# rhysnewell/Lorikeet

Hardware: AMD Instinct MI355X
Metric: PairHMM cell-updates/s (GCUPS) (higher is better)
Workload: dtype f64; 1 GPU; config2 x 1024 regions per GPU: 128 reads x 8 haps, R=150, H=300; regions_per_gpu=1024, seed=1000, env=PHMM_REGION_OWN_QUEUE=0 in this process only

## Files before the change

### lorikeet_amd/csrc/phmm_chain_kernels.hip

```cpp
#include "phmm_device.hpp"

namespace phmm {

namespace {

#ifndef PHMM_CHAIN_L
#define PHMM_CHAIN_L 16
#endif
constexpr int CL = PHMM_CHAIN_L;
#ifndef PHMM_RING
#define PHMM_RING 256
#endif
constexpr int RING = PHMM_RING;
constexpr int RING_SLOTS = RING + 4 + 1;
constexpr int CHAIN_META = CHAIN_MAX_READS + 8;
constexpr uint32_t X_PAD = 0x100u;
constexpr uint32_t X_NONE = 0x102u;
constexpr int LEAD = CL - 1;

__device__ __forceinline__ double from_left_inject(double v, double inject, bool group_head) {
    constexpr int ctrl = CL == 16 ? 0x111 : 0x138;
    int lo = __builtin_amdgcn_update_dpp(__double2loint(inject), __double2loint(v), ctrl, 0xf, 0xf, false);
    int hi = __builtin_amdgcn_update_dpp(__double2hiint(inject), __double2hiint(v), ctrl, 0xf, 0xf, false);
    if constexpr (CL == 32) {
        lo = group_head ? __double2loint(inject) : lo;
        hi = group_head ? __double2hiint(inject) : hi;
    }
    return __hiloint2double(hi, lo);
}

template <int K>
__device__ __forceinline__ void chain_fallback(const ForwardParams &p, const ChainItem &it, RowConst *ring, int lane,
                                               int grp, int l, const HapCols<K> &hc, int H, bool hv, int a, int Nh) {
    const uint32_t reg = it.region;
    for (uint32_t r = it.read_begin; r < it.read_end; ++r) {
        const uint32_t ro = p.read_off[r];
        const int R = (int)(p.read_off[r + 1] - ro);
        bool z = false;
        for (int row = lane; row < R; row += WAVE) z |= row_blocks_prescale(p, ro + row);
        const bool scaled = __ballot(z) == 0ull;
        const bool staged = R + 1 <= RING;
        lds_wave_sync();
        if (staged) {
            if (lane == 0) ring[0] = neutral_row();
            for (int row = lane; row < R; row += WAVE) ring[row + 1] = make_row(p, ro, row, R, scaled);
        }
        lds_wave_sync();
        const double scale0 = (scaled && R > 0) ? 1.0 - p.eps[p.gcp[ro]] : 1.0;
        const double fin = (scaled && R > 0) ? 1.0 - p.eps[p.base_q[ro + R - 1]] : 1.0;
        const double c0 = p.initial_condition / (double)H * scale0;
        const bool group_head = (CL == 32) && (lane == 32);
        double s = staged ? sweep_general<CL, K>(LdsView{ring}, R, l, group_head, hc, H, c0, scaled, fin)
                          : sweep_general<CL, K>(GlobalRowView{p, ro, R, scaled}, R, l, group_head, hc, H, c0, scaled, fin);
#pragma unroll
        for (int off = CL / 2; off > 0; off >>= 1) s += __shfl_xor(s, off, WAVE);
        if (l == 0 && hv) {
            const double v = log10(s) - p.initial_condition_log10;
            p.out[p.out_off[reg] + (uint64_t)(r - p.region_read_off[reg]) * (uint64_t)Nh + a] = v;
            if (const uint32_t sb = status_bits(v)) atomicOr(p.status, sb);
        }
    }
    (void)grp;
}

template <int K>
__device__ __forceinline__ void chain_fallback_streams(const ForwardParams &p, uint32_t reg, uint32_t r_begin, int n_mine,
                                                       int n_iter, int lane, int l, const HapCols<K> &hc, int H, bool hv,
                                                       int a, int Nh) {
    const uint64_t group_bits = 0xffffull << (lane & ~15);
    for (int i = 0; i < n_iter; ++i) {
        const bool valid = i < n_mine;
        const uint32_t r = r_begin + (uint32_t)i;
        const uint32_t ro = valid ? p.read_off[r] : 0u;
        const int R = valid ? (int)(p.read_off[r + 1] - ro) : 0;
        bool z = false;
        for (int row = l; row < R; row += 16) z |= row_blocks_prescale(p, ro + row);
        const bool scaled = (__ballot(z) & group_bits) == 0ull;
        const double scale0 = (scaled && R > 0) ? 1.0 - p.eps[p.gcp[ro]] : 1.0;
        const double fin = (scaled && R > 0) ? 1.0 - p.eps[p.base_q[ro + R - 1]] : 1.0;
        const double c0 = p.initial_condition / (double)H * scale0;
        double s = sweep_general<16, K>(GlobalRowView{p, ro, R, scaled}, R, l, false, hc, H, c0, scaled, fin);
#pragma unroll
        for (int off = 8; off > 0; off >>= 1) s += __shfl_xor(s, off, WAVE);
        if (l == 0 && hv && valid) {
            const double v = log10(s) - p.initial_condition_log10;
            p.out[p.out_off[reg] + (uint64_t)(r - p.region_read_off[reg]) * (uint64_t)Nh + a] = v;
            if (const uint32_t sb = status_bits(v)) atomicOr(p.status, sb);
        }
    }
}

}

template <int CLT, int K, int MODE = CHAIN_PLAIN>
__device__ __forceinline__ void chain_body(const ForwardParams &p, const ChainItem it, unsigned char *smem, const ChainItemX *x = nullptr,
                                           double *park = nullptr) {
    static_assert(CLT == CL, "one lanes-per-pair value per compilation unit");
    static_assert(MODE == CHAIN_PLAIN || CL == 16, "prefix sharing: 16 lanes per pair");
    const int col0 = MODE == CHAIN_SUFFIX ? (int)x->mask_or_col0 : 0;
    const uint32_t park_rows = MODE == CHAIN_PLAIN ? 0u : 16u * x->park_rows16;
    const uint32_t park_mask = MODE == CHAIN_PARK ? (uint32_t)x->mask_or_col0 : 0u;
    const int lane = threadIdx.x;
    const int grp = lane / CL, l = lane % CL;
    const bool group_head = (CL == 32) && (lane == 32);
    const uint32_t reg = it.region;
    const int n_chain = (int)(it.read_end - it.read_begin);
    const uint32_t h0 = p.region_hap_off[reg];
    const int Nh = (int)(p.region_hap_off[reg + 1] - h0);
    const int S = (CL == 16) ? (int)it.streams : 1;
    const int GS = (WAVE / CL) / S;
    const int sid = grp / GS;
    const int a = MODE == CHAIN_PLAIN ? (int)it.quad * GS + grp % GS : (int)x->hap[grp & 3];
    const bool hv = a < Nh;
    const int n_sub = (n_chain + S - 1) / S;
    const int TPS = (RING / 4) / S;
    const int NM = RING / S - 1;
    auto n_of = [&](int s) { return max(0, min(n_sub, n_chain - s * n_sub)); };
    const int n_mine = n_of(sid);
    uint32_t ho = 0;
    int H = 0;
    if (hv) {
        ho = p.hap_off[h0 + a];
        H = (int)(p.hap_off[h0 + a + 1] - ho);
    }
    RowConst *ring = reinterpret_cast<RowConst *>(smem);
    uint32_t *roff = reinterpret_cast<uint32_t *>(ring + RING_SLOTS);
    uint32_t *stot = roff + CHAIN_META;

    HapCols<K> hc;
    bool lane_n = false;
#pragma unroll
    for (int w = 0; w < HapCols<K>::W; ++w) hc.y[w] = 0u;
#pragma unroll
    for (int k = 0; k < K; ++k) {
        const int col = col0 + l * K + k;
        uint32_t y = col < H ? (uint32_t)p.hap_bases[ho + col] : X_PAD;
        const bool is_n = (y == 'N');
        lane_n |= is_n;
        hc.set(k, y);
    }

    const uint32_t rb = it.read_begin;
    const uint32_t byte0 = p.read_off[rb];
    const uint32_t bytes = p.read_off[it.read_end] - byte0;
    bool z = false;
    for (uint32_t i = lane; i < bytes; i += WAVE) z |= row_blocks_prescale(p, byte0 + i);
    if ((__ballot(z) | __ballot(lane_n)) != 0ull) {
        if constexpr (MODE == CHAIN_SUFFIX) {
            for (uint32_t r = rb + (uint32_t)l; r < it.read_end && hv; r += CL)
                p.out[p.out_off[reg] + (uint64_t)(r - p.region_read_off[reg]) * (uint64_t)Nh + a] = __longlong_as_double(0x7ff8000000000000ll);
            if (lane == 0) atomicOr(p.status, STATUS_RESCUE);
            return;
        }
        if (S == 1)
            chain_fallback<K>(p, it, ring, lane, grp, l, hc, H, hv, a, Nh);
        else if constexpr (CL == 16)
            chain_fallback_streams<K>(p, reg, rb + (uint32_t)(sid * n_sub), n_mine, n_sub, lane, l, hc, H, hv, a, Nh);
        return;
    }
    {
        const int sj = lane / n_sub, ij = lane % n_sub;
        uint32_t len = lane < n_chain ? p.read_off[rb + lane + 1] - p.read_off[rb + lane] + 2u : 0u;
        uint32_t incl = len;
#pragma unroll
        for (int off = 1; off < WAVE; off <<= 1) {
            const uint32_t v = __shfl_up(incl, off, WAVE);
            if (lane >= off) incl += v;
        }
        const uint32_t before = __shfl(incl, max(sj * n_sub - 1, 0), WAVE);
        const int cb = sj * (n_sub + 1);
        if (lane < 4) stot[lane] = 0u;
        if (lane < n_chain) {
            roff[cb + ij] = p.read_off[rb + lane];
            if (ij + 1 == n_of(sj)) {
                roff[cb + ij + 1] = p.read_off[rb + lane + 1];
                stot[sj] = incl - (sj > 0 ? before : 0u);
            }
        }
        if (lane == 0) ring[RING_SLOTS - 1] = neutral_row();
    }
    lds_wave_sync();
    const int S_max = (int)max(max(stot[0], stot[1]), max(stot[2], stot[3]));
    const double c_unit = ldexp(1.0, 1010);

    uint32_t pb_x = 0, pb_q = 0, pb_qp = 0, pb_i = 0, pb_d = 0, pb_dp = 0, pb_g = 0, pb_gn = 0;
    double pb_bM = 0.0, pb_bD = 0.0;
    int p_Q = 0;
    const bool producer = lane < S * TPS;
    const int ps = producer ? lane / TPS : 0, pj = lane % TPS;
    const int pcb = ps * (n_sub + 1), pn = n_of(ps);
    int p_lo = 0, p_row = pj - LEAD - TPS;
    p_Q = pj - TPS;
    uint32_t p_ro = pn > 0 ? roff[pcb] : 0u;
    int p_R = pn > 0 ? (int)(roff[pcb + 1] - p_ro) : 0;
    auto advance = [&]() {
        p_row += TPS;
        p_Q += TPS;
        while (p_lo < pn && p_row >= p_R + 2) {
            p_row -= p_R + 2;
            ++p_lo;
            if (p_lo < pn) {
                p_ro = roff[pcb + p_lo];
                p_R = (int)(roff[pcb + p_lo + 1] - p_ro);
            }
        }
    };
    auto issue = [&]() {
        advance();
        const int row = p_row, R = p_R;
        const uint32_t ro = p_ro;
        if constexpr (MODE == CHAIN_SUFFIX) {
            if (producer && p_lo < pn && row >= 0 && (uint32_t)p_Q < park_rows) {
                const double *at = park + 2 * ((size_t)x->park_row0 + (size_t)p_Q);
                pb_bM = at[0];
                pb_bD = at[1];
            }
        }
        if (producer && p_lo < pn && row >= 0 && row <= R) {
            pb_qp = row > 0 ? (uint32_t)p.base_q[ro + row - 1] : 0u;
            if (row < R) {
                pb_x = p.read_bases[ro + row];
                pb_q = p.base_q[ro + row];
                pb_i = p.ins_q[ro + row];
                pb_d = p.del_q[ro + row];
                pb_dp = row > 0 ? (uint32_t)p.del_q[ro + row - 1] : 0u;
                pb_g = p.gcp[ro + row];
                pb_gn = row + 1 < R ? (uint32_t)p.gcp[ro + row + 1] : 0u;
            }
        }
    };
    auto finish = [&](int Q0) {
        const int Q = Q0 + pj;
        const int lo = p_lo, row = p_row, R = p_R;
        RowConst n;
        if (lo < pn && row >= 0) {
            if (row < R) {
                n = make_row_bytes(p, pb_x, pb_q, pb_qp, pb_i, pb_d, pb_dp, pb_g, pb_gn, row == 0, row + 1 >= R, true);
            } else if (row == R) {
                n.mm = 1.0 - p.eps[pb_qp]; n.bI = n.mm; n.gI = 1.0; n.dDp = 0.0; n.dd = 1.0; n.pm = 1.0; n.px = 1.0;
                n.x = X_PAD; n.pad0 = (uint32_t)lo; n.pad1 = 0.0;
            } else {
                n.mm = 0.0; n.bI = 0.0; n.gI = 0.0; n.dDp = 0.0; n.dd = 1.0; n.pm = 0.0; n.px = 0.0;
                n.x = X_NONE; n.pad0 = 0;
                n.pad1 = c_unit * (lo + 1 < pn ? 1.0 - p.eps[p.gcp[roff[pcb + lo + 1]]] : 1.0);
            }
            if constexpr (MODE == CHAIN_SUFFIX) {
                n.pm = pb_bM;
                n.pad1 = pb_bD;
            }
        } else {
            n = neutral_row();
        }
        if (producer) {
            const int slot = ps * (NM + 2) + (Q & NM);
            ring[slot] = n;
            if ((Q & NM) == 0) ring[slot + NM + 1] = n;
        }
    };
    issue();
    finish(0);
    issue();
    finish(TPS);
    issue();
    finish(2 * TPS);
    lds_wave_sync();
    issue();

    const double c0 = c_unit * (n_mine > 0 ? 1.0 - p.eps[p.gcp[roff[sid * (n_sub + 1)]]] : 1.0);
    double Mp[K], Ip[K], Dp[K];
#pragma unroll
    for (int k = 0; k < K; ++k) {
        Mp[k] = 0.0;
        Ip[k] = 0.0;
        Dp[k] = c0;
    }
    double aM, aI, aD, bM = 0.0, bI = 0.0, bD = c0;
    const int edge_lane = (H > col0 ? H - 1 - col0 : 0) / K, edge_k = (H > col0 ? H - 1 - col0 : 0) % K;
    const bool last_lane = (l == edge_lane);
    const uint32_t sum_code = last_lane ? X_PAD : 0xffffffffu;
    const double log10_scale = log10(c_unit) + log10((double)H);
    auto emit = [&](const RowConst &c) {
        {
            if (last_lane && c.x == X_PAD && hv) {
                const uint32_t r = rb + (uint32_t)(sid * n_sub) + c.pad0;
                int ek = edge_k;
                asm volatile("" : "+v"(ek));
                double sum = 0.0;
#pragma unroll
                for (int k = 0; k < K; ++k)
                    if (k == ek) sum = (Dp[k] + Mp[k]) + Ip[k];
                const double v = log10(sum) - log10_scale;
                p.out[p.out_off[reg] + (uint64_t)(r - p.region_read_off[reg]) * (uint64_t)Nh + a] = v;
                if (const uint32_t sb = status_bits(v)) atomicOr(p.status, sb);
            }
        }
    };

    int q = LEAD - l;
    const int my_ring = sid * (NM + 2);
    const uint32_t my_rows = (uint32_t)(uintptr_t)(ring + my_ring);
    RowConst cA = lds_row(ring, my_ring + (q & NM)), cB;
    int q1 = q + 1;
    const int T = (S_max + CL - 1 + 1) & ~1;
    bool park_lane = false;
    double2 *park_at = nullptr;
    if constexpr (MODE == CHAIN_PARK) {
        park_lane = grp == 0 && ((park_mask >> l) & 1u) != 0u && hv && (uint32_t)(q + T) <= park_rows;
        const int b = __popc(park_mask & ((1u << l) - 1u));
        park_at = reinterpret_cast<double2 *>(park) + ((size_t)x->park_row0 + (size_t)b * park_rows + (size_t)q);
    }
    const int phase = (int)((blockIdx.x * 2654435761u) >> 26) & (TPS - 2);
    for (int t0 = 0, t1 = min(T, TPS - phase), tick = 0; t0 < T; t0 = t1, t1 = min(T, t1 + TPS), ++tick) {
        if (tick >= 1) {
            finish(TPS * tick + 2 * TPS);
            lds_wave_sync();
            issue();
        }
        for (int t = t0; t < t1; t += 2) {
            uint32_t pair_at;
            asm("v_mad_u32_u24 %0, %1, %2, %3" : "=v"(pair_at) : "v"((uint32_t)(q1 & NM)), "s"((uint32_t)sizeof(RowConst)), "v"(my_rows));
            cB = lds_row_at(pair_at, 0);
            if constexpr (MODE == CHAIN_SUFFIX) {
                aI = from_left_inject(Ip[K - 1], fma(bM, cA.bI, bI * cA.gI), group_head);
                aM = from_left_inject(Mp[K - 1], cA.pm, group_head);
            } else {
                aM = from_left<CL>(Mp[K - 1], group_head);
                aI = from_left<CL>(Ip[K - 1], group_head);
            }
            aD = from_left_inject(Dp[K - 1], cA.pad1, group_head);
            row_update<K, ROW_FAST_EXEC>(Mp, Ip, Dp, bM, bI, bD, aM, aD, cA, hc, 1.0);
            if constexpr (MODE == CHAIN_PARK)
                if (park_lane) park_at[0] = make_double2(Mp[K - 1], Dp[K - 1]);
            if (__ballot(cA.x == sum_code) != 0ull) emit(cA);
            cA = lds_row_at(pair_at, 1);
            if constexpr (MODE == CHAIN_SUFFIX) {
                bI = from_left_inject(Ip[K - 1], fma(aM, cB.bI, aI * cB.gI), group_head);
                bM = from_left_inject(Mp[K - 1], cB.pm, group_head);
            } else {
                bM = from_left<CL>(Mp[K - 1], group_head);
                bI = from_left<CL>(Ip[K - 1], group_head);
            }
            bD = from_left_inject(Dp[K - 1], cB.pad1, group_head);
            row_update<K, ROW_FAST_EXEC>(Mp, Ip, Dp, aM, aI, aD, bM, bD, cB, hc, 1.0);
            if constexpr (MODE == CHAIN_PARK) {
                if (park_lane) park_at[1] = make_double2(Mp[K - 1], Dp[K - 1]);
                park_at += 2;
            }
            if (__ballot(cB.x == sum_code) != 0ull) emit(cB);
            q1 += 2;
        }
    }
}


#define PHMM_CHAIN_K_LIST(X) \
    X(2) X(3) X(4) X(5) X(6) X(7) X(8) X(9) X(10) X(11) X(12) X(13) X(14) X(15) X(16) X(17) X(18) X(19) X(20) X(21) X(22) \
    X(23) X(24) X(25)

template <int CLT, int KLO, int KHI>
__global__ __launch_bounds__(WAVE, 2) void phmm_forward_chain(const ChainParams cp) {
    extern __shared__ __attribute__((aligned(16))) unsigned char smem[];
    const ChainItem it = cp.items[blockIdx.x];
    switch (__builtin_amdgcn_readfirstlane((int)it.k)) {
#define PHMM_CASE(KK)                                                  \
    case KK:                                                           \
        if constexpr (KK >= KLO && KK <= KHI) chain_body<CLT, KK>(cp.f, it, smem); \
        break;
        PHMM_CHAIN_K_LIST(PHMM_CASE)
#undef PHMM_CASE
        default:
            break;
    }
}

template <int CLT, int K>
__global__ __launch_bounds__(WAVE, 2) void phmm_forward_chain_k(const ChainParams cp) {
    extern __shared__ __attribute__((aligned(16))) unsigned char smem[];
    chain_body<CLT, K>(cp.f, cp.items[blockIdx.x], smem);
}

#define PHMM_CHAIN_CAT2(a, b) a##b
#define PHMM_CHAIN_CAT(a, b) PHMM_CHAIN_CAT2(a, b)
#define PHMM_CHAIN_LAUNCH PHMM_CHAIN_CAT(launch_chain_L, PHMM_CHAIN_L)

hipError_t PHMM_CHAIN_LAUNCH(int single_k, const ChainParams &cp, hipStream_t stream) {
    const size_t lds = (size_t)RING_SLOTS * sizeof(RowConst) + (CHAIN_META + 4) * sizeof(uint32_t);
#define PHMM_CASE(KK)                                                                                     \
    if (single_k == KK) {                                                                                 \
        hipLaunchKernelGGL((phmm_forward_chain_k<CL, KK>), dim3(cp.n_items), dim3(WAVE), lds, stream, cp); \
        return hipGetLastError();                                                                         \
    }
    PHMM_CHAIN_K_LIST(PHMM_CASE)
#undef PHMM_CASE
#define PHMM_RANGE(R, LO, HI)                                                                                       \
    if (single_k == -(R + 1)) {                                                                                     \
        hipLaunchKernelGGL((phmm_forward_chain<CL, LO, HI>), dim3(cp.n_items), dim3(WAVE), lds, stream, cp);        \
        return hipGetLastError();                                                                                   \
    }
    PHMM_CHAIN_RANGES(PHMM_RANGE)
#undef PHMM_RANGE
    return hipErrorInvalidValue;
}

#if PHMM_CHAIN_L == 16
hipError_t launch_chain_L32(int single_k, const ChainParams &cp, hipStream_t stream);
hipError_t launch_chain_L64(int single_k, const ChainParams &cp, hipStream_t stream);
int chain_max_k() { return 25; }
hipError_t launch_chain(int L, int single_k, const ChainParams &cp, hipStream_t stream) {
    if (!cp.n_items) return hipSuccess;
    return L == 16 ? launch_chain_L16(single_k, cp, stream) : L == 32 ? launch_chain_L32(single_k, cp, stream)
         : L == 64 ? launch_chain_L64(single_k, cp, stream) : hipErrorInvalidValue;
}
#endif

}
```

Baseline: 4555 GCUPS.

## Batch chain result emission into per-lane parked slots and flush once per wave

Row-end results are no longer written immediately with a divergent log10 and global store per emission. Each result's sum and tag are now compacted into per-lane registers via readlane, and the whole batch is flushed when the slots fill or the chain ends. The flush does the log10, the output store and the status atomic across many lanes in one go. When all active lanes share the same edge column, a uniform switch selects the column directly instead of scanning all K columns. The aim is to take serialized epilogue work out of the inner recurrence loop, at the cost of extra registers, readlane sequences and some added code size.

```diff
diff --git a/lorikeet_amd/csrc/phmm_chain_kernels.hip b/lorikeet_amd/csrc/phmm_chain_kernels.hip
--- a/lorikeet_amd/csrc/phmm_chain_kernels.hip
+++ b/lorikeet_amd/csrc/phmm_chain_kernels.hip
@@ -17,6 +17,10 @@
 constexpr uint32_t X_PAD = 0x100u;
 constexpr uint32_t X_NONE = 0x102u;
 constexpr int LEAD = CL - 1;
+constexpr int PARK_SLOTS = WAVE;
+constexpr size_t CHAIN_LDS = (size_t)RING_SLOTS * sizeof(RowConst) + (CHAIN_META + 4) * sizeof(uint32_t);
+static_assert(8 * CHAIN_LDS <= 160 * 1024, "two waves per SIMD");
+static_assert(CHAIN_MAX_READS <= 64, "a parked result names its read in six bits");
 
 __device__ __forceinline__ double from_left_inject(double v, double inject, bool group_head) {
     constexpr int ctrl = CL == 16 ? 0x111 : 0x138;
@@ -91,6 +95,10 @@
 }
 
 }
+
+#define PHMM_CHAIN_K_LIST(X) \
+    X(2) X(3) X(4) X(5) X(6) X(7) X(8) X(9) X(10) X(11) X(12) X(13) X(14) X(15) X(16) X(17) X(18) X(19) X(20) X(21) X(22) \
+    X(23) X(24) X(25)
 
 template <int CLT, int K, int MODE = CHAIN_PLAIN>
 __device__ __forceinline__ void chain_body(const ForwardParams &p, const ChainItem it, unsigned char *smem, const ChainItemX *x = nullptr,
@@ -277,23 +285,70 @@
     double aM, aI, aD, bM = 0.0, bI = 0.0, bD = c0;
     const int edge_lane = (H > col0 ? H - 1 - col0 : 0) / K, edge_k = (H > col0 ? H - 1 - col0 : 0) % K;
     const bool last_lane = (l == edge_lane);
-    const uint32_t sum_code = last_lane ? X_PAD : 0xffffffffu;
+    const uint32_t sum_code = (last_lane && hv) ? X_PAD : 0xffffffffu;
     const double log10_scale = log10(c_unit) + log10((double)H);
-    auto emit = [&](const RowConst &c) {
-        {
-            if (last_lane && c.x == X_PAD && hv) {
-                const uint32_t r = rb + (uint32_t)(sid * n_sub) + c.pad0;
+    int edge_uni = -1;
+    if (const uint64_t hvm = __ballot(hv)) {
+        const int e0 = __builtin_amdgcn_readlane(edge_k, (int)__builtin_ctzll(hvm));
+        if (__ballot(hv && edge_k != e0) == 0ull) edge_uni = e0;
+    }
+    int n_parked = 0;
+    uint32_t park_lo = 0u, park_hi = 0u, park_tag = 0u;
+    const uint32_t tag0 = ((uint32_t)grp << 6) + (uint32_t)(sid * n_sub);
+    auto flush = [&]() {
+        const bool mine = lane < n_parked;
+        const uint32_t tag = mine ? park_tag : 0u;
+        const double sum = mine ? __hiloint2double((int)park_hi, (int)park_lo) : 1.0;
+        const int src = (int)(tag >> 6) * CL;
+        const int sa = __shfl(a, src, WAVE);
+        const double ls = __shfl(log10_scale, src, WAVE);
+        if (mine) {
+            const uint32_t r = rb + (tag & 63u);
+            const double v = log10(sum) - ls;
+            p.out[p.out_off[reg] + (uint64_t)(r - p.region_read_off[reg]) * (uint64_t)Nh + sa] = v;
+            if (const uint32_t sb = status_bits(v)) atomicOr(p.status, sb);
+        }
+        n_parked = 0;
+    };
+    auto emit = [&](const RowConst &c, uint64_t em) {
+        double sum = 0.0;
+        if (c.x == sum_code) {
+            if (edge_uni >= 0) {
+                switch (edge_uni) {
+#define PHMM_CASE(KK)                                                    \
+    case KK:                                                             \
+        if constexpr (KK < K) sum = (Dp[KK] + Mp[KK]) + Ip[KK];          \
+        break;
+                    PHMM_CASE(0) PHMM_CASE(1) PHMM_CHAIN_K_LIST(PHMM_CASE)
+#undef PHMM_CASE
+                    default:
+                        break;
+                }
+            } else {
                 int ek = edge_k;
                 asm volatile("" : "+v"(ek));
-                double sum = 0.0;
+                double sd = 0.0, sm = 0.0, si = 0.0;
 #pragma unroll
                 for (int k = 0; k < K; ++k)
-                    if (k == ek) sum = (Dp[k] + Mp[k]) + Ip[k];
-                const double v = log10(sum) - log10_scale;
-                p.out[p.out_off[reg] + (uint64_t)(r - p.region_read_off[reg]) * (uint64_t)Nh + a] = v;
-                if (const uint32_t sb = status_bits(v)) atomicOr(p.status, sb);
-            }
-        }
+                    if (k == ek) {
+                        sd = Dp[k];
+                        sm = Mp[k];
+                        si = Ip[k];
+                    }
+                sum = (sd + sm) + si;
+            }
+        }
+        const uint32_t s_lo = (uint32_t)__double2loint(sum), s_hi = (uint32_t)__double2hiint(sum), s_tag = tag0 + c.pad0;
+        do {
+            const int src = (int)__builtin_ctzll(em);
+            const bool here = lane == n_parked;
+            park_lo = here ? (uint32_t)__builtin_amdgcn_readlane(s_lo, src) : park_lo;
+            park_hi = here ? (uint32_t)__builtin_amdgcn_readlane(s_hi, src) : park_hi;
+            park_tag = here ? (uint32_t)__builtin_amdgcn_readlane(s_tag, src) : park_tag;
+            ++n_parked;
+            em &= em - 1;
+        } while (em);
+        if (n_parked > PARK_SLOTS - WAVE / CL) flush();
     };
 
     int q = LEAD - l;
@@ -331,7 +386,7 @@
             row_update<K, ROW_FAST_EXEC>(Mp, Ip, Dp, bM, bI, bD, aM, aD, cA, hc, 1.0);
             if constexpr (MODE == CHAIN_PARK)
                 if (park_lane) park_at[0] = make_double2(Mp[K - 1], Dp[K - 1]);
-            if (__ballot(cA.x == sum_code) != 0ull) emit(cA);
+            if (const uint64_t em = __ballot(cA.x == sum_code)) emit(cA, em);
             cA = lds_row_at(pair_at, 1);
             if constexpr (MODE == CHAIN_SUFFIX) {
                 bI = from_left_inject(Ip[K - 1], fma(aM, cB.bI, aI * cB.gI), group_head);
@@ -346,16 +401,14 @@
                 if (park_lane) park_at[1] = make_double2(Mp[K - 1], Dp[K - 1]);
                 park_at += 2;
             }
-            if (__ballot(cB.x == sum_code) != 0ull) emit(cB);
+            if (const uint64_t em = __ballot(cB.x == sum_code)) emit(cB, em);
             q1 += 2;
         }
     }
-}
-
-
-#define PHMM_CHAIN_K_LIST(X) \
-    X(2) X(3) X(4) X(5) X(6) X(7) X(8) X(9) X(10) X(11) X(12) X(13) X(14) X(15) X(16) X(17) X(18) X(19) X(20) X(21) X(22) \
-    X(23) X(24) X(25)
+    if (n_parked > 0) flush();
+}
+
+
 
 template <int CLT, int KLO, int KHI>
 __global__ __launch_bounds__(WAVE, 2) void phmm_forward_chain(const ChainParams cp) {
@@ -384,7 +437,7 @@
 #define PHMM_CHAIN_LAUNCH PHMM_CHAIN_CAT(launch_chain_L, PHMM_CHAIN_L)
 
 hipError_t PHMM_CHAIN_LAUNCH(int single_k, const ChainParams &cp, hipStream_t stream) {
-    const size_t lds = (size_t)RING_SLOTS * sizeof(RowConst) + (CHAIN_META + 4) * sizeof(uint32_t);
+    const size_t lds = CHAIN_LDS;
 #define PHMM_CASE(KK)                                                                                     \
     if (single_k == KK) {                                                                                 \
         hipLaunchKernelGGL((phmm_forward_chain_k<CL, KK>), dim3(cp.n_items), dim3(WAVE), lds, stream, cp); \
```

Result: no change. 4546 GCUPS (-0.2%).
